# palash1992/GEM

Measured on NVIDIA H100. Metric: nodes/sec embedded at d=128, higher is better.
Workload: dtype f32

## Files before the change

gem_b200/csrc/apply_tc.cu:

```cuda
#include "tc_common.cuh"

namespace gemb {

struct ApplyTcParams {
    int64_t n;
    const float *Q;
    const float *M;
    float *Out;
    int b1, b2, ldm, ldo;
    uint32_t a_lbo;
    uint32_t a_tile;
    uint32_t b_tile;
    uint32_t raw_slot;
};

template <int TILE_M, int NPAD>
__global__ void __launch_bounds__(384, 1) apply_tc_kernel(ApplyTcParams p) {
    extern __shared__ __align__(128) char smem[];
    __shared__ __align__(8) uint64_t s_full[2], s_tile_full, s_tile_free;
    const int tid = threadIdx.x, lane = tid & 31, warp = tid >> 5;
    const int kchunks = p.b1 / 4;
    const int ksteps = p.b1 / 8;
    const uint32_t a_sbo = 128u;
    const uint32_t b_lbo = 128u;
    const uint32_t b_sbo = (uint32_t)kchunks * 128u;
    char *raw_base = smem;
    char *a_hi = smem + 2 * (size_t)p.raw_slot, *a_lo = a_hi + p.a_tile;
    char *b_hi = a_lo + p.a_tile, *b_lo = b_hi + p.b_tile;

    if (tid == 0) {
        for (int i = 0; i < 2; i++) tc::mbar_init(tc::smem_u32(&s_full[i]), 1);
        tc::mbar_init(tc::smem_u32(&s_tile_full), 4);
        tc::mbar_init(tc::smem_u32(&s_tile_free), 8);
        asm volatile("fence.mbarrier_init.release.cluster;" ::: "memory");
    }
    for (int idx = tid; idx < NPAD * kchunks; idx += blockDim.x) {
        const int nn = idx % NPAD, kc = idx / NPAD;
        float4 v = make_float4(0.f, 0.f, 0.f, 0.f);
        if (nn < p.b2) {
            const float *m = p.M + (size_t)(4 * kc) * p.ldm + nn;
            v = make_float4(__ldg(m), __ldg(m + p.ldm), __ldg(m + 2 * (size_t)p.ldm), __ldg(m + 3 * (size_t)p.ldm));
        }
        uint4 hi, lo;
        tc::split_tf32(v, hi, lo);
        const uint32_t off = (uint32_t)(nn >> 3) * b_sbo + (uint32_t)(nn & 7) * 16u + (uint32_t)kc * b_lbo;
        *(uint4 *)(b_hi + off) = hi;
        *(uint4 *)(b_lo + off) = lo;
    }
    tc::fence_proxy_async();
    __syncthreads();

    const int64_t tiles_total = (p.n + TILE_M - 1) / TILE_M;
    const int nt = (int)((tiles_total - blockIdx.x + gridDim.x - 1) / gridDim.x);
    auto tile_row0 = [&](int t) { return ((int64_t)blockIdx.x + (int64_t)t * gridDim.x) * TILE_M; };
    auto tile_rows = [&](int t) { const int64_t r0 = tile_row0(t); return (int)(p.n - r0 < TILE_M ? p.n - r0 : TILE_M); };

    if (warp >= 8) {
        auto issue = [&](int t) {
            const int slot = t & 1;
            const uint32_t bytes = (uint32_t)tile_rows(t) * (uint32_t)p.b1 * 4u;
            const uint32_t bar = tc::smem_u32(&s_full[slot]);
            tc::mbar_expect_tx(bar, bytes);
            tc::bulk_g2s(tc::smem_u32(raw_base + (size_t)slot * p.raw_slot), p.Q + tile_row0(t) * p.b1, bytes, bar);
        };
        if (tid == 256) {
            if (nt > 0) issue(0);
            if (nt > 1) issue(1);
        }
        const int ltid = tid - 256;
        for (int t = 0; t < nt; t++) {
            const int slot = t & 1;
            const char *raw = raw_base + (size_t)slot * p.raw_slot;
            tc::mbar_wait(tc::smem_u32(&s_full[slot]), (uint32_t)(t >> 1) & 1);
            if (t >= 1) tc::mbar_wait(tc::smem_u32(&s_tile_free), (uint32_t)(t - 1) & 1);
            const int vr = tile_rows(t);
            for (int idx = ltid; idx < TILE_M * kchunks; idx += 128) {
                const int m = idx / kchunks, kc = idx - m * kchunks;
                float4 v = make_float4(0.f, 0.f, 0.f, 0.f);
                if (m < vr) v = *(const float4 *)(raw + ((size_t)m * p.b1 + 4 * kc) * 4);
                uint4 hi, lo;
                tc::split_tf32(v, hi, lo);
                const uint32_t off = (uint32_t)(m >> 3) * a_sbo + (uint32_t)(m & 7) * 16u + (uint32_t)kc * p.a_lbo;
                *(uint4 *)(a_hi + off) = hi;
                *(uint4 *)(a_lo + off) = lo;
            }
            tc::fence_proxy_async();
            __syncwarp();
            if (lane == 0) tc::mbar_arrive(tc::smem_u32(&s_tile_full));
            tc::named_sync(1, 128);
            if (tid == 256 && t + 2 < nt) issue(t + 2);
        }
    } else {
        const int wg = warp >> 2;
        const bool active = wg * 64 < TILE_M;
        float acc[NPAD / 2];
        const uint32_t a_off = (uint32_t)wg * 8u * a_sbo;
        for (int t = 0; t < nt; t++) {
            tc::mbar_wait(tc::smem_u32(&s_tile_full), (uint32_t)t & 1);
            __syncwarp();
            uint64_t dah = tc::make_desc(tc::smem_u32(a_hi) + a_off, p.a_lbo, a_sbo), dal = tc::make_desc(tc::smem_u32(a_lo) + a_off, p.a_lbo, a_sbo);
            uint64_t dbh = tc::make_desc(tc::smem_u32(b_hi), b_lbo, b_sbo), dbl = tc::make_desc(tc::smem_u32(b_lo), b_lbo, b_sbo);
            const uint64_t a_step = (uint64_t)((2u * p.a_lbo) >> 4), b_step = (uint64_t)((2u * b_lbo) >> 4);
            if (active) {
                tc::wgmma_fence();
                for (int ks = 0; ks < ksteps; ks++) {
                    tc::wgmma_tf32<NPAD>(acc, dah, dbh, ks > 0 ? 1u : 0u);
                    tc::wgmma_tf32<NPAD>(acc, dah, dbl, 1u);
                    tc::wgmma_tf32<NPAD>(acc, dal, dbh, 1u);
                    dah += a_step; dal += a_step; dbh += b_step; dbl += b_step;
                }
                tc::wgmma_commit();
                tc::wgmma_wait_all();
            }
            __syncwarp();
            if (lane == 0) tc::mbar_arrive(tc::smem_u32(&s_tile_free));
            if (!active) continue;
            const int vr = tile_rows(t);
            const int r0 = wg * 64 + (warp & 3) * 16 + (lane >> 2);
            float *orow = p.Out + tile_row0(t) * p.ldo;
#pragma unroll
            for (int j = 0; j < NPAD / 8; j++) {
                const int col = j * 8 + (lane & 3) * 2;
                if (col < p.b2) {
                    if (r0 < vr) *(float2 *)(orow + (size_t)r0 * p.ldo + col) = make_float2(acc[4 * j], acc[4 * j + 1]);
                    if (r0 + 8 < vr) *(float2 *)(orow + (size_t)(r0 + 8) * p.ldo + col) = make_float2(acc[4 * j + 2], acc[4 * j + 3]);
                }
            }
        }
    }
}

template <int TILE_M, int NPAD>
static int apply_tc_launch_t(gemb_ctx *ctx, const ApplyTcParams &p, int grid, size_t smem_bytes) {
    static size_t attr_bytes = 0;
    if (attr_bytes < smem_bytes) {
        GEMB_CUDA(cudaFuncSetAttribute(apply_tc_kernel<TILE_M, NPAD>, cudaFuncAttributeMaxDynamicSharedMemorySize, (int)smem_bytes));
        attr_bytes = smem_bytes;
    }
    apply_tc_kernel<TILE_M, NPAD><<<grid, 384, smem_bytes, ctx->stream>>>(p);
    GEMB_CUDA(cudaGetLastError());
    count_launch();
    return GEMB_OK;
}

template <int TILE_M>
static int apply_tc_dispatch(gemb_ctx *ctx, const ApplyTcParams &p, int npad, int grid, size_t smem_bytes) {
    switch (npad) {
        case 32: return apply_tc_launch_t<TILE_M, 32>(ctx, p, grid, smem_bytes);
        case 64: return apply_tc_launch_t<TILE_M, 64>(ctx, p, grid, smem_bytes);
        case 80: return apply_tc_launch_t<TILE_M, 80>(ctx, p, grid, smem_bytes);
        case 96: return apply_tc_launch_t<TILE_M, 96>(ctx, p, grid, smem_bytes);
        default: return apply_tc_launch_t<TILE_M, 128>(ctx, p, grid, smem_bytes);
    }
}

static int pad_width(int b) {
    const int widths[5] = {32, 64, 80, 96, 128};
    for (int w : widths) if (w >= b) return w;
    return 128;
}

static size_t apply_smem_bytes(int tile_m, int b1, int npad) {
    const size_t raw_slot = (size_t)tile_m * b1 * 4, a_tile = (size_t)(b1 / 4) * (16 * tile_m + 16);
    const size_t b_tile = (size_t)(npad / 8) * (b1 / 4) * 128;
    return 2 * raw_slot + 2 * a_tile + 2 * b_tile + 256;
}

int apply_tc_launch(gemb_ctx *ctx, int64_t n, const float *Q, int b1, const float *M, int ldm, int b2, float *Out, int ldo) {
    if (b1 % 8 || b2 % 4 || b1 > 128 || ldo < b2 || ldo % 4 || ((uintptr_t)Out & 15) || n <= 0) return GEMB_ERR_UNSUPPORTED;
    const int cfg[5][2] = {{128, 128}, {64, 128}, {128, 64}, {64, 64}, {64, 32}};
    int tile_m = 0, nbw = 0;
    for (const auto &c : cfg) {
        const int w = std::min(c[1], b2);
        if (apply_smem_bytes(c[0], b1, pad_width(w)) <= 226 * 1024) { tile_m = c[0]; nbw = w; break; }
    }
    if (!tile_m) return GEMB_ERR_UNSUPPORTED;
    const int64_t tiles = (n + tile_m - 1) / tile_m;
    int grid = ctx->sm_count;
    if (grid > tiles) grid = (int)tiles;
    for (int n0 = 0; n0 < b2; n0 += nbw) {
        ApplyTcParams p;
        const int w = std::min(nbw, b2 - n0), npad = pad_width(w);
        p.n = n; p.Q = Q; p.M = M + n0; p.Out = Out + n0; p.b1 = b1; p.b2 = w; p.ldm = ldm; p.ldo = ldo;
        p.a_lbo = 16u * (uint32_t)tile_m + 16u;
        p.a_tile = (uint32_t)(b1 / 4) * p.a_lbo;
        p.b_tile = (uint32_t)(npad / 8) * (uint32_t)(b1 / 4) * 128u;
        p.raw_slot = (uint32_t)((size_t)tile_m * b1 * 4);
        const size_t smem_bytes = apply_smem_bytes(tile_m, b1, npad);
        if (tile_m == 128) GEMB_TRY(apply_tc_dispatch<128>(ctx, p, npad, grid, smem_bytes));
        else GEMB_TRY(apply_tc_dispatch<64>(ctx, p, npad, grid, smem_bytes));
    }
    return GEMB_OK;
}

}
```

gem_b200/csrc/gram_tc.cu:

```cuda
#include "tc_common.cuh"

namespace gemb {

struct GramTcParams {
    int64_t n;
    const float *P, *Q;
    int ldp, ldq;
    int m0, n0, mb, nb;
    double *part;
    int ldg;
    int64_t part_stride;
    int stage_rows;
    uint32_t tile_bytes_a, tile_bytes_b;
    uint32_t raw_bytes_p, raw_bytes_q;
};

__device__ __forceinline__ void transform_unit(const char *raw, int ld, int c0, int w, int valid_rows, int k4, int j32,
                                               int lane, char *tile_hi, char *tile_lo, uint32_t lbo, uint32_t sbo) {
    const int mn = j32 * 32 + lane;
    if (mn >= w) return;
    const int k0 = k4 * 4;
    const float *src = (const float *)raw + (size_t)k0 * ld + c0 + mn;
    float4 v;
    v.x = (k0 + 0 < valid_rows) ? src[0] : 0.f;
    v.y = (k0 + 1 < valid_rows) ? src[(size_t)ld] : 0.f;
    v.z = (k0 + 2 < valid_rows) ? src[2 * (size_t)ld] : 0.f;
    v.w = (k0 + 3 < valid_rows) ? src[3 * (size_t)ld] : 0.f;
    uint4 hi, lo;
    tc::split_tf32(v, hi, lo);
    const uint32_t off = (uint32_t)(mn >> 3) * sbo + (uint32_t)(mn & 7) * 16u + (uint32_t)k4 * lbo;
    *(uint4 *)(tile_hi + off) = hi;
    *(uint4 *)(tile_lo + off) = lo;
}

template <bool QRAW, bool BSEP, int NPAD>
__global__ void __launch_bounds__(384, 1) gram_tc_kernel(GramTcParams p) {
    extern __shared__ __align__(128) char smem[];
    __shared__ __align__(8) uint64_t s_full[3], s_tile_full[2], s_tile_free[2];
    const int tid = threadIdx.x, lane = tid & 31, warp = tid >> 5;
    const int kblocks = p.stage_rows / 8;
    const int kquads = p.stage_rows / 4;
    const uint32_t lbo = 128u;
    const uint32_t sbo = (uint32_t)kquads * 128u;
    const uint32_t raw_stage = p.raw_bytes_p + (QRAW ? p.raw_bytes_q : 0);
    const uint32_t stage_bytes = 2 * p.tile_bytes_a + (BSEP ? 2 * p.tile_bytes_b : 0);
    char *raw_base = smem;
    char *tile_base = smem + 3 * (size_t)raw_stage;

    if (tid == 0) {
        for (int i = 0; i < 2; i++) { tc::mbar_init(tc::smem_u32(&s_tile_full[i]), 4); tc::mbar_init(tc::smem_u32(&s_tile_free[i]), 8); }
        for (int i = 0; i < 3; i++) tc::mbar_init(tc::smem_u32(&s_full[i]), 1);
        asm volatile("fence.mbarrier_init.release.cluster;" ::: "memory");
    }
    __syncthreads();

    const int64_t stages_total = (p.n + p.stage_rows - 1) / p.stage_rows;
    const int64_t per_cta = (stages_total + gridDim.x - 1) / gridDim.x;
    const int64_t s_begin = (int64_t)blockIdx.x * per_cta;
    const int64_t s_end = s_begin + per_cta < stages_total ? s_begin + per_cta : stages_total;
    const int nst = (int)(s_end > s_begin ? s_end - s_begin : 0);

    if (warp >= 8) {
        const int lw = warp - 8;
        auto issue = [&](int it) {
            const int slot = it % 3;
            const int64_t row0 = (s_begin + it) * p.stage_rows;
            const int64_t vr = p.n - row0 < p.stage_rows ? p.n - row0 : p.stage_rows;
            const uint32_t bytes_p = (uint32_t)(vr * p.ldp * 4), bytes_q = QRAW ? (uint32_t)(vr * p.ldq * 4) : 0u;
            const uint32_t bar = tc::smem_u32(&s_full[slot]);
            char *dst = raw_base + (size_t)slot * raw_stage;
            tc::mbar_expect_tx(bar, bytes_p + bytes_q);
            tc::bulk_g2s(tc::smem_u32(dst), p.P + row0 * p.ldp, bytes_p, bar);
            if (QRAW) tc::bulk_g2s(tc::smem_u32(dst + p.raw_bytes_p), p.Q + row0 * p.ldq, bytes_q, bar);
        };
        if (tid == 256)
            for (int it = 0; it < 3 && it < nst; it++) issue(it);
        for (int it = 0; it < nst; it++) {
            const int st = it & 1, slot = it % 3;
            char *base = tile_base + (size_t)st * stage_bytes;
            const char *raw = raw_base + (size_t)slot * raw_stage;
            tc::mbar_wait(tc::smem_u32(&s_full[slot]), (uint32_t)(it / 3) & 1);
            if (it >= 2) tc::mbar_wait(tc::smem_u32(&s_tile_free[st]), (uint32_t)((it >> 1) - 1) & 1);
            const int64_t row0 = (s_begin + it) * p.stage_rows;
            const int vr = (int)(p.n - row0 < p.stage_rows ? p.n - row0 : p.stage_rows);
            const int units_a = kquads * ((p.mb + 31) / 32);
#pragma unroll 3
            for (int u = lw; u < units_a; u += 4)
                transform_unit(raw, p.ldp, p.m0, p.mb, vr, u % kquads, u / kquads, lane, base, base + p.tile_bytes_a, lbo, sbo);
            if (BSEP) {
                const int units_b = kquads * ((p.nb + 31) / 32);
                char *qb = base + 2 * p.tile_bytes_a;
                const char *rb = QRAW ? raw + p.raw_bytes_p : raw;
                const int ldb = QRAW ? p.ldq : p.ldp;
#pragma unroll 3
                for (int u = lw; u < units_b; u += 4)
                    transform_unit(rb, ldb, p.n0, p.nb, vr, u % kquads, u / kquads, lane, qb, qb + p.tile_bytes_b, lbo, sbo);
            }
            tc::fence_proxy_async();
            __syncwarp();
            if (lane == 0) tc::mbar_arrive(tc::smem_u32(&s_tile_full[st]));
            tc::named_sync(1, 128);
            if (tid == 256 && it + 3 < nst) issue(it + 3);
        }
    } else {
        const int wg = warp >> 2;
        const bool active = wg * 64 < p.mb;
        float acc[NPAD / 2], racc[NPAD / 2];
#pragma unroll
        for (int i = 0; i < NPAD / 2; i++) racc[i] = 0.f;
        for (int it = 0; it < nst; it++) {
            const int st = it & 1;
            tc::mbar_wait(tc::smem_u32(&s_tile_full[st]), (uint32_t)(it >> 1) & 1);
            if (active) {
                const uint32_t a_hi = tc::smem_u32(tile_base + (size_t)st * stage_bytes), a_lo = a_hi + p.tile_bytes_a;
                const uint32_t b_hi = BSEP ? a_hi + 2 * p.tile_bytes_a : a_hi;
                const uint32_t b_lo = BSEP ? b_hi + p.tile_bytes_b : a_lo;
                const uint32_t a_off = (uint32_t)wg * 8u * sbo;
                uint64_t dah = tc::make_desc(a_hi + a_off, lbo, sbo), dal = tc::make_desc(a_lo + a_off, lbo, sbo);
                uint64_t dbh = tc::make_desc(b_hi, lbo, sbo), dbl = tc::make_desc(b_lo, lbo, sbo);
                const uint64_t step = (uint64_t)((2u * lbo) >> 4);
                tc::wgmma_fence();
                for (int kb = 0; kb < kblocks; kb++) {
                    tc::wgmma_tf32<NPAD>(acc, dah, dbh, kb > 0 ? 1u : 0u);
                    tc::wgmma_tf32<NPAD>(acc, dah, dbl, 1u);
                    tc::wgmma_tf32<NPAD>(acc, dal, dbh, 1u);
                    dah += step; dal += step; dbh += step; dbl += step;
                }
                tc::wgmma_commit();
                tc::wgmma_wait_all();
            }
            __syncwarp();
            if (lane == 0) tc::mbar_arrive(tc::smem_u32(&s_tile_free[st]));
            if (active) {
#pragma unroll
                for (int i = 0; i < NPAD / 2; i++) racc[i] += acc[i];
            }
        }
        if (active) {
            const int r0 = wg * 64 + (warp & 3) * 16 + (lane >> 2);
            double *dst = p.part + (size_t)blockIdx.x * p.part_stride + (size_t)p.m0 * p.ldg + p.n0;
#pragma unroll
            for (int i = 0; i < NPAD / 2; i++) {
                const int row = r0 + ((i >> 1) & 1) * 8, col = (i >> 2) * 8 + (lane & 3) * 2 + (i & 1);
                if (row < p.mb && col < p.nb) dst[(size_t)row * p.ldg + col] = (double)racc[i];
            }
        }
    }
}

template <bool QRAW, bool BSEP, int NPAD>
static int gram_tc_launch_t(gemb_ctx *ctx, const GramTcParams &p, int grid, size_t smem_bytes) {
    static size_t attr_bytes = 0;
    if (attr_bytes < smem_bytes) {
        GEMB_CUDA(cudaFuncSetAttribute(gram_tc_kernel<QRAW, BSEP, NPAD>, cudaFuncAttributeMaxDynamicSharedMemorySize, (int)smem_bytes));
        attr_bytes = smem_bytes;
    }
    gram_tc_kernel<QRAW, BSEP, NPAD><<<grid, 384, smem_bytes, ctx->stream>>>(p);
    GEMB_CUDA(cudaGetLastError());
    count_launch();
    return GEMB_OK;
}

template <bool QRAW, bool BSEP>
static int gram_tc_dispatch(gemb_ctx *ctx, const GramTcParams &p, int grid, size_t smem_bytes) {
    if (p.nb <= 32) return gram_tc_launch_t<QRAW, BSEP, 32>(ctx, p, grid, smem_bytes);
    if (p.nb <= 64) return gram_tc_launch_t<QRAW, BSEP, 64>(ctx, p, grid, smem_bytes);
    if (p.nb <= 80) return gram_tc_launch_t<QRAW, BSEP, 80>(ctx, p, grid, smem_bytes);
    if (p.nb <= 96) return gram_tc_launch_t<QRAW, BSEP, 96>(ctx, p, grid, smem_bytes);
    return gram_tc_launch_t<QRAW, BSEP, 128>(ctx, p, grid, smem_bytes);
}

int gram_tc_launch(gemb_ctx *ctx, int64_t n, const float *P, int b1, const float *Q, int b2, double *G) {
    const bool cross = (P != Q);
    if (b1 % 4 || b2 % 4 || n <= 0) return GEMB_ERR_UNSUPPORTED;
    const int bm = (b1 + 127) / 128, bn = (b2 + 127) / 128;
    const size_t cols_raw = (size_t)b1 + (cross ? b2 : 0);
    size_t cols_tile = 0;
    for (int i = 0; i < bm; i++)
        for (int j = 0; j < bn; j++) {
            const int mb = std::min(128, b1 - 128 * i), nb = std::min(128, b2 - 128 * j);
            const bool bsep = cross || i != j;
            cols_tile = std::max(cols_tile, (size_t)(mb + 7) / 8 * 8 + (bsep ? (size_t)(nb + 7) / 8 * 8 : 0));
        }
    const size_t bytes_per_row = 3 * 4 * cols_raw + 2 * 2 * 4 * cols_tile;
    int rows = (int)((176 * 1024) / bytes_per_row) / 8 * 8;
    if (rows > 64) rows = 64;
    if (rows < 8) return GEMB_ERR_UNSUPPORTED;
    const size_t sbo = (size_t)(rows / 4) * 128;
    const size_t raw_stage = (size_t)rows * cols_raw * 4;
    const size_t smem_bytes = 3 * raw_stage + 2 * cols_tile / 8 * 2 * sbo + 16 * sbo + 1024;
    if (smem_bytes > 226 * 1024) return GEMB_ERR_UNSUPPORTED;
    const int64_t stages_total = (n + rows - 1) / rows;
    int grid = ctx->sm_count;
    if (grid > stages_total) grid = (int)stages_total;
    double *part = nullptr;
    GEMB_TRY(red_scratch(ctx, (size_t)grid * b1 * b2, &part));
    GramTcParams p;
    p.n = n; p.P = P; p.Q = Q; p.ldp = b1; p.ldq = b2;
    p.part = part; p.ldg = b2; p.part_stride = (int64_t)b1 * b2;
    p.stage_rows = rows;
    p.raw_bytes_p = (uint32_t)(rows * b1 * 4);
    p.raw_bytes_q = (uint32_t)(rows * b2 * 4);
    for (int i = 0; i < bm; i++)
        for (int j = 0; j < bn; j++) {
            p.m0 = 128 * i; p.mb = std::min(128, b1 - p.m0);
            p.n0 = 128 * j; p.nb = std::min(128, b2 - p.n0);
            p.tile_bytes_a = (uint32_t)((p.mb + 7) / 8) * (uint32_t)(rows / 4) * 128u;
            p.tile_bytes_b = (uint32_t)((p.nb + 7) / 8) * (uint32_t)(rows / 4) * 128u;
            if (cross) GEMB_TRY((gram_tc_dispatch<true, true>(ctx, p, grid, smem_bytes)));
            else if (i != j) GEMB_TRY((gram_tc_dispatch<false, true>(ctx, p, grid, smem_bytes)));
            else GEMB_TRY((gram_tc_dispatch<false, false>(ctx, p, grid, smem_bytes)));
        }
    return sum_partials_launch(ctx, grid, (int64_t)b1 * b2, part, G);
}

}
```

gem_b200/csrc/tc_common.cuh:

```cuda
#pragma once
#include "common.cuh"

namespace gemb {
namespace tc {

__device__ __forceinline__ uint32_t smem_u32(const void *p) { return (uint32_t)__cvta_generic_to_shared(p); }

__device__ __forceinline__ void mbar_init(uint32_t bar, uint32_t count) {
    asm volatile("mbarrier.init.shared::cta.b64 [%0], %1;" ::"r"(bar), "r"(count));
}
__device__ __forceinline__ bool mbar_try_wait(uint32_t bar, uint32_t parity) {
    uint32_t ok;
    asm volatile(
        "{\n.reg .pred p;\nmbarrier.try_wait.parity.shared::cta.b64 p, [%1], %2;\nselp.b32 %0, 1, 0, p;\n}"
        : "=r"(ok)
        : "r"(bar), "r"(parity)
        : "memory");
    return ok != 0;
}
__device__ __forceinline__ void mbar_wait(uint32_t bar, uint32_t parity) {
    for (uint32_t it = 0; it < (1u << 22); it++) {
        if (mbar_try_wait(bar, parity)) return;
        __nanosleep(40);
    }
    __trap();
}
__device__ __forceinline__ void mbar_arrive(uint32_t bar) {
    asm volatile("mbarrier.arrive.shared::cta.b64 _, [%0];" ::"r"(bar) : "memory");
}
__device__ __forceinline__ void mbar_expect_tx(uint32_t bar, uint32_t bytes) {
    asm volatile("mbarrier.arrive.expect_tx.shared::cta.b64 _, [%0], %1;" ::"r"(bar), "r"(bytes) : "memory");
}
__device__ __forceinline__ void bulk_g2s(uint32_t dst_smem, const void *src, uint32_t bytes, uint32_t bar) {
    asm volatile("cp.async.bulk.shared::cluster.global.mbarrier::complete_tx::bytes [%0], [%1], %2, [%3];"
                 ::"r"(dst_smem), "l"(src), "r"(bytes), "r"(bar) : "memory");
}
__device__ __forceinline__ void fence_proxy_async() { asm volatile("fence.proxy.async.shared::cta;" ::: "memory"); }
__device__ __forceinline__ void named_sync(uint32_t id, uint32_t count) {
    asm volatile("bar.sync %0, %1;" ::"r"(id), "r"(count) : "memory");
}

__device__ __forceinline__ uint32_t to_tf32(float x) {
    uint32_t r;
    asm("cvt.rna.tf32.f32 %0, %1;" : "=r"(r) : "f"(x));
    return r;
}
__device__ __forceinline__ void split_tf32(const float4 &v, uint4 &hi, uint4 &lo) {
    hi.x = to_tf32(v.x); hi.y = to_tf32(v.y); hi.z = to_tf32(v.z); hi.w = to_tf32(v.w);
    lo.x = to_tf32(v.x - __uint_as_float(hi.x));
    lo.y = to_tf32(v.y - __uint_as_float(hi.y));
    lo.z = to_tf32(v.z - __uint_as_float(hi.z));
    lo.w = to_tf32(v.w - __uint_as_float(hi.w));
}

__device__ __forceinline__ uint64_t make_desc(uint32_t smem_addr, uint32_t lbo_bytes, uint32_t sbo_bytes) {
    uint64_t d = 0;
    d |= (uint64_t)((smem_addr >> 4) & 0x3FFF);
    d |= (uint64_t)((lbo_bytes >> 4) & 0x3FFF) << 16;
    d |= (uint64_t)((sbo_bytes >> 4) & 0x3FFF) << 32;
    return d;
}

__device__ __forceinline__ void wgmma_fence() { asm volatile("wgmma.fence.sync.aligned;" ::: "memory"); }
__device__ __forceinline__ void wgmma_commit() { asm volatile("wgmma.commit_group.sync.aligned;" ::: "memory"); }
__device__ __forceinline__ void wgmma_wait_all() { asm volatile("wgmma.wait_group.sync.aligned 0;" ::: "memory"); }

template <int N> __device__ __forceinline__ void wgmma_tf32(float (&d)[N / 2], uint64_t a, uint64_t b, uint32_t scale_d);
template <> __device__ __forceinline__ void wgmma_tf32<32>(float (&d)[16], uint64_t a, uint64_t b, uint32_t scale_d) {
    asm volatile(
        "{\n.reg .pred p;\nsetp.ne.b32 p, %18, 0;\n"
        "wgmma.mma_async.sync.aligned.m64n32k8.f32.tf32.tf32 {"
        "%0, %1, %2, %3, %4, %5, %6, %7, %8, %9, %10, %11, %12, %13, %14, %15"
        "}, %16, %17, p, 1, 1;\n}\n"
        : "+f"(d[0]), "+f"(d[1]), "+f"(d[2]), "+f"(d[3]), "+f"(d[4]), "+f"(d[5]), "+f"(d[6]), "+f"(d[7]),
          "+f"(d[8]), "+f"(d[9]), "+f"(d[10]), "+f"(d[11]), "+f"(d[12]), "+f"(d[13]), "+f"(d[14]), "+f"(d[15])
        : "l"(a), "l"(b), "r"(scale_d));
}
template <> __device__ __forceinline__ void wgmma_tf32<64>(float (&d)[32], uint64_t a, uint64_t b, uint32_t scale_d) {
    asm volatile(
        "{\n.reg .pred p;\nsetp.ne.b32 p, %34, 0;\n"
        "wgmma.mma_async.sync.aligned.m64n64k8.f32.tf32.tf32 {"
        "%0, %1, %2, %3, %4, %5, %6, %7, %8, %9, %10, %11, %12, %13, %14, %15, "
        "%16, %17, %18, %19, %20, %21, %22, %23, %24, %25, %26, %27, %28, %29, %30, %31"
        "}, %32, %33, p, 1, 1;\n}\n"
        : "+f"(d[0]), "+f"(d[1]), "+f"(d[2]), "+f"(d[3]), "+f"(d[4]), "+f"(d[5]), "+f"(d[6]), "+f"(d[7]),
          "+f"(d[8]), "+f"(d[9]), "+f"(d[10]), "+f"(d[11]), "+f"(d[12]), "+f"(d[13]), "+f"(d[14]), "+f"(d[15]),
          "+f"(d[16]), "+f"(d[17]), "+f"(d[18]), "+f"(d[19]), "+f"(d[20]), "+f"(d[21]), "+f"(d[22]), "+f"(d[23]),
          "+f"(d[24]), "+f"(d[25]), "+f"(d[26]), "+f"(d[27]), "+f"(d[28]), "+f"(d[29]), "+f"(d[30]), "+f"(d[31])
        : "l"(a), "l"(b), "r"(scale_d));
}
template <> __device__ __forceinline__ void wgmma_tf32<80>(float (&d)[40], uint64_t a, uint64_t b, uint32_t scale_d) {
    asm volatile(
        "{\n.reg .pred p;\nsetp.ne.b32 p, %42, 0;\n"
        "wgmma.mma_async.sync.aligned.m64n80k8.f32.tf32.tf32 {"
        "%0, %1, %2, %3, %4, %5, %6, %7, %8, %9, %10, %11, %12, %13, %14, %15, "
        "%16, %17, %18, %19, %20, %21, %22, %23, %24, %25, %26, %27, %28, %29, %30, %31, "
        "%32, %33, %34, %35, %36, %37, %38, %39"
        "}, %40, %41, p, 1, 1;\n}\n"
        : "+f"(d[0]), "+f"(d[1]), "+f"(d[2]), "+f"(d[3]), "+f"(d[4]), "+f"(d[5]), "+f"(d[6]), "+f"(d[7]),
          "+f"(d[8]), "+f"(d[9]), "+f"(d[10]), "+f"(d[11]), "+f"(d[12]), "+f"(d[13]), "+f"(d[14]), "+f"(d[15]),
          "+f"(d[16]), "+f"(d[17]), "+f"(d[18]), "+f"(d[19]), "+f"(d[20]), "+f"(d[21]), "+f"(d[22]), "+f"(d[23]),
          "+f"(d[24]), "+f"(d[25]), "+f"(d[26]), "+f"(d[27]), "+f"(d[28]), "+f"(d[29]), "+f"(d[30]), "+f"(d[31]),
          "+f"(d[32]), "+f"(d[33]), "+f"(d[34]), "+f"(d[35]), "+f"(d[36]), "+f"(d[37]), "+f"(d[38]), "+f"(d[39])
        : "l"(a), "l"(b), "r"(scale_d));
}
template <> __device__ __forceinline__ void wgmma_tf32<96>(float (&d)[48], uint64_t a, uint64_t b, uint32_t scale_d) {
    asm volatile(
        "{\n.reg .pred p;\nsetp.ne.b32 p, %50, 0;\n"
        "wgmma.mma_async.sync.aligned.m64n96k8.f32.tf32.tf32 {"
        "%0, %1, %2, %3, %4, %5, %6, %7, %8, %9, %10, %11, %12, %13, %14, %15, "
        "%16, %17, %18, %19, %20, %21, %22, %23, %24, %25, %26, %27, %28, %29, %30, %31, "
        "%32, %33, %34, %35, %36, %37, %38, %39, %40, %41, %42, %43, %44, %45, %46, %47"
        "}, %48, %49, p, 1, 1;\n}\n"
        : "+f"(d[0]), "+f"(d[1]), "+f"(d[2]), "+f"(d[3]), "+f"(d[4]), "+f"(d[5]), "+f"(d[6]), "+f"(d[7]),
          "+f"(d[8]), "+f"(d[9]), "+f"(d[10]), "+f"(d[11]), "+f"(d[12]), "+f"(d[13]), "+f"(d[14]), "+f"(d[15]),
          "+f"(d[16]), "+f"(d[17]), "+f"(d[18]), "+f"(d[19]), "+f"(d[20]), "+f"(d[21]), "+f"(d[22]), "+f"(d[23]),
          "+f"(d[24]), "+f"(d[25]), "+f"(d[26]), "+f"(d[27]), "+f"(d[28]), "+f"(d[29]), "+f"(d[30]), "+f"(d[31]),
          "+f"(d[32]), "+f"(d[33]), "+f"(d[34]), "+f"(d[35]), "+f"(d[36]), "+f"(d[37]), "+f"(d[38]), "+f"(d[39]),
          "+f"(d[40]), "+f"(d[41]), "+f"(d[42]), "+f"(d[43]), "+f"(d[44]), "+f"(d[45]), "+f"(d[46]), "+f"(d[47])
        : "l"(a), "l"(b), "r"(scale_d));
}
template <> __device__ __forceinline__ void wgmma_tf32<128>(float (&d)[64], uint64_t a, uint64_t b, uint32_t scale_d) {
    asm volatile(
        "{\n.reg .pred p;\nsetp.ne.b32 p, %66, 0;\n"
        "wgmma.mma_async.sync.aligned.m64n128k8.f32.tf32.tf32 {"
        "%0, %1, %2, %3, %4, %5, %6, %7, %8, %9, %10, %11, %12, %13, %14, %15, "
        "%16, %17, %18, %19, %20, %21, %22, %23, %24, %25, %26, %27, %28, %29, %30, %31, "
        "%32, %33, %34, %35, %36, %37, %38, %39, %40, %41, %42, %43, %44, %45, %46, %47, "
        "%48, %49, %50, %51, %52, %53, %54, %55, %56, %57, %58, %59, %60, %61, %62, %63"
        "}, %64, %65, p, 1, 1;\n}\n"
        : "+f"(d[0]), "+f"(d[1]), "+f"(d[2]), "+f"(d[3]), "+f"(d[4]), "+f"(d[5]), "+f"(d[6]), "+f"(d[7]),
          "+f"(d[8]), "+f"(d[9]), "+f"(d[10]), "+f"(d[11]), "+f"(d[12]), "+f"(d[13]), "+f"(d[14]), "+f"(d[15]),
          "+f"(d[16]), "+f"(d[17]), "+f"(d[18]), "+f"(d[19]), "+f"(d[20]), "+f"(d[21]), "+f"(d[22]), "+f"(d[23]),
          "+f"(d[24]), "+f"(d[25]), "+f"(d[26]), "+f"(d[27]), "+f"(d[28]), "+f"(d[29]), "+f"(d[30]), "+f"(d[31]),
          "+f"(d[32]), "+f"(d[33]), "+f"(d[34]), "+f"(d[35]), "+f"(d[36]), "+f"(d[37]), "+f"(d[38]), "+f"(d[39]),
          "+f"(d[40]), "+f"(d[41]), "+f"(d[42]), "+f"(d[43]), "+f"(d[44]), "+f"(d[45]), "+f"(d[46]), "+f"(d[47]),
          "+f"(d[48]), "+f"(d[49]), "+f"(d[50]), "+f"(d[51]), "+f"(d[52]), "+f"(d[53]), "+f"(d[54]), "+f"(d[55]),
          "+f"(d[56]), "+f"(d[57]), "+f"(d[58]), "+f"(d[59]), "+f"(d[60]), "+f"(d[61]), "+f"(d[62]), "+f"(d[63])
        : "l"(a), "l"(b), "r"(scale_d));
}

}
}
```

Measured before the change: 14.89 million.

## Widen loader warps, deepen raw staging, add tail-8 wgmma path and n72 tile

For tiles of width 96 or less, the apply and gram kernels now use 8 loader warps instead of 4, so the TF32 hi/lo split transform gets more threads. The gram kernel sizes its raw TMA staging ring from the shared memory left over, up to 8 slots instead of a fixed 3. It also rewrites the transform loop as a flat strided item walk. When mb is 65..72, the second warpgroup computes the 8-row tail with swapped m64n8 wgmmas instead of a full 64-row tile, and a new n72 instantiation reduces padding waste. These changes add register pressure and more code paths, and the tail path has subtle index and store logic.

```diff
diff --git a/gem_b200/csrc/apply_tc.cu b/gem_b200/csrc/apply_tc.cu
--- a/gem_b200/csrc/apply_tc.cu
+++ b/gem_b200/csrc/apply_tc.cu
@@ -14,8 +14,11 @@
     uint32_t raw_slot;
 };
 
+__host__ __device__ constexpr int apply_loader_warps(int npad) { return npad <= 96 ? 8 : 4; }
+
 template <int TILE_M, int NPAD>
-__global__ void __launch_bounds__(384, 1) apply_tc_kernel(ApplyTcParams p) {
+__global__ void __launch_bounds__(256 + 32 * apply_loader_warps(NPAD), 1) apply_tc_kernel(ApplyTcParams p) {
+    constexpr int LW = apply_loader_warps(NPAD);
     extern __shared__ __align__(128) char smem[];
     __shared__ __align__(8) uint64_t s_full[2], s_tile_full, s_tile_free;
     const int tid = threadIdx.x, lane = tid & 31, warp = tid >> 5;
@@ -30,7 +33,7 @@
 
     if (tid == 0) {
         for (int i = 0; i < 2; i++) tc::mbar_init(tc::smem_u32(&s_full[i]), 1);
-        tc::mbar_init(tc::smem_u32(&s_tile_full), 4);
+        tc::mbar_init(tc::smem_u32(&s_tile_full), LW);
         tc::mbar_init(tc::smem_u32(&s_tile_free), 8);
         asm volatile("fence.mbarrier_init.release.cluster;" ::: "memory");
     }
@@ -74,7 +77,7 @@
             tc::mbar_wait(tc::smem_u32(&s_full[slot]), (uint32_t)(t >> 1) & 1);
             if (t >= 1) tc::mbar_wait(tc::smem_u32(&s_tile_free), (uint32_t)(t - 1) & 1);
             const int vr = tile_rows(t);
-            for (int idx = ltid; idx < TILE_M * kchunks; idx += 128) {
+            for (int idx = ltid; idx < TILE_M * kchunks; idx += 32 * LW) {
                 const int m = idx / kchunks, kc = idx - m * kchunks;
                 float4 v = make_float4(0.f, 0.f, 0.f, 0.f);
                 if (m < vr) v = *(const float4 *)(raw + ((size_t)m * p.b1 + 4 * kc) * 4);
@@ -87,7 +90,7 @@
             tc::fence_proxy_async();
             __syncwarp();
             if (lane == 0) tc::mbar_arrive(tc::smem_u32(&s_tile_full));
-            tc::named_sync(1, 128);
+            tc::named_sync(1, 32 * LW);
             if (tid == 256 && t + 2 < nt) issue(t + 2);
         }
     } else {
@@ -137,7 +140,7 @@
         GEMB_CUDA(cudaFuncSetAttribute(apply_tc_kernel<TILE_M, NPAD>, cudaFuncAttributeMaxDynamicSharedMemorySize, (int)smem_bytes));
         attr_bytes = smem_bytes;
     }
-    apply_tc_kernel<TILE_M, NPAD><<<grid, 384, smem_bytes, ctx->stream>>>(p);
+    apply_tc_kernel<TILE_M, NPAD><<<grid, 256 + 32 * apply_loader_warps(NPAD), smem_bytes, ctx->stream>>>(p);
     GEMB_CUDA(cudaGetLastError());
     count_launch();
     return GEMB_OK;
diff --git a/gem_b200/csrc/gram_tc.cu b/gem_b200/csrc/gram_tc.cu
--- a/gem_b200/csrc/gram_tc.cu
+++ b/gem_b200/csrc/gram_tc.cu
@@ -11,32 +11,42 @@
     int ldg;
     int64_t part_stride;
     int stage_rows;
+    int nraw;
     uint32_t tile_bytes_a, tile_bytes_b;
     uint32_t raw_bytes_p, raw_bytes_q;
 };
 
-__device__ __forceinline__ void transform_unit(const char *raw, int ld, int c0, int w, int valid_rows, int k4, int j32,
-                                               int lane, char *tile_hi, char *tile_lo, uint32_t lbo, uint32_t sbo) {
-    const int mn = j32 * 32 + lane;
-    if (mn >= w) return;
-    const int k0 = k4 * 4;
-    const float *src = (const float *)raw + (size_t)k0 * ld + c0 + mn;
-    float4 v;
-    v.x = (k0 + 0 < valid_rows) ? src[0] : 0.f;
-    v.y = (k0 + 1 < valid_rows) ? src[(size_t)ld] : 0.f;
-    v.z = (k0 + 2 < valid_rows) ? src[2 * (size_t)ld] : 0.f;
-    v.w = (k0 + 3 < valid_rows) ? src[3 * (size_t)ld] : 0.f;
-    uint4 hi, lo;
-    tc::split_tf32(v, hi, lo);
-    const uint32_t off = (uint32_t)(mn >> 3) * sbo + (uint32_t)(mn & 7) * 16u + (uint32_t)k4 * lbo;
-    *(uint4 *)(tile_hi + off) = hi;
-    *(uint4 *)(tile_lo + off) = lo;
-}
-
-template <bool QRAW, bool BSEP, int NPAD>
-__global__ void __launch_bounds__(384, 1) gram_tc_kernel(GramTcParams p) {
+__device__ __forceinline__ void transform_items(const char *raw, int ld, int c0, int w, int kquads, int valid_rows, int t,
+                                                int nt, char *tile_hi, char *tile_lo, uint32_t lbo, uint32_t sbo) {
+    const int dm = nt % w, dk = nt / w;
+    int mn = t % w, k4 = t / w;
+#pragma unroll 2
+    for (; k4 < kquads;) {
+        const int k0 = k4 * 4;
+        const float *src = (const float *)raw + (size_t)k0 * ld + c0 + mn;
+        float4 v;
+        v.x = (k0 + 0 < valid_rows) ? src[0] : 0.f;
+        v.y = (k0 + 1 < valid_rows) ? src[(size_t)ld] : 0.f;
+        v.z = (k0 + 2 < valid_rows) ? src[2 * (size_t)ld] : 0.f;
+        v.w = (k0 + 3 < valid_rows) ? src[3 * (size_t)ld] : 0.f;
+        uint4 hi, lo;
+        tc::split_tf32(v, hi, lo);
+        const uint32_t off = (uint32_t)(mn >> 3) * sbo + (uint32_t)(mn & 7) * 16u + (uint32_t)k4 * lbo;
+        *(uint4 *)(tile_hi + off) = hi;
+        *(uint4 *)(tile_lo + off) = lo;
+        mn += dm; k4 += dk;
+        if (mn >= w) { mn -= w; k4++; }
+    }
+}
+
+constexpr int GRAM_MAX_RAW = 8;
+__host__ __device__ constexpr int gram_loader_warps(int npad) { return npad <= 96 ? 8 : 4; }
+
+template <bool QRAW, bool BSEP, int NPAD, bool TAIL8>
+__global__ void __launch_bounds__(256 + 32 * gram_loader_warps(NPAD), 1) gram_tc_kernel(GramTcParams p) {
+    constexpr int LW = gram_loader_warps(NPAD);
     extern __shared__ __align__(128) char smem[];
-    __shared__ __align__(8) uint64_t s_full[3], s_tile_full[2], s_tile_free[2];
+    __shared__ __align__(8) uint64_t s_full[GRAM_MAX_RAW], s_tile_full[2], s_tile_free[2];
     const int tid = threadIdx.x, lane = tid & 31, warp = tid >> 5;
     const int kblocks = p.stage_rows / 8;
     const int kquads = p.stage_rows / 4;
@@ -45,11 +55,12 @@
     const uint32_t raw_stage = p.raw_bytes_p + (QRAW ? p.raw_bytes_q : 0);
     const uint32_t stage_bytes = 2 * p.tile_bytes_a + (BSEP ? 2 * p.tile_bytes_b : 0);
     char *raw_base = smem;
-    char *tile_base = smem + 3 * (size_t)raw_stage;
+    const int nraw = p.nraw;
+    char *tile_base = smem + (size_t)nraw * raw_stage;
 
     if (tid == 0) {
-        for (int i = 0; i < 2; i++) { tc::mbar_init(tc::smem_u32(&s_tile_full[i]), 4); tc::mbar_init(tc::smem_u32(&s_tile_free[i]), 8); }
-        for (int i = 0; i < 3; i++) tc::mbar_init(tc::smem_u32(&s_full[i]), 1);
+        for (int i = 0; i < 2; i++) { tc::mbar_init(tc::smem_u32(&s_tile_full[i]), LW); tc::mbar_init(tc::smem_u32(&s_tile_free[i]), 8); }
+        for (int i = 0; i < nraw; i++) tc::mbar_init(tc::smem_u32(&s_full[i]), 1);
         asm volatile("fence.mbarrier_init.release.cluster;" ::: "memory");
     }
     __syncthreads();
@@ -61,9 +72,8 @@
     const int nst = (int)(s_end > s_begin ? s_end - s_begin : 0);
 
     if (warp >= 8) {
-        const int lw = warp - 8;
         auto issue = [&](int it) {
-            const int slot = it % 3;
+            const int slot = it % nraw;
             const int64_t row0 = (s_begin + it) * p.stage_rows;
             const int64_t vr = p.n - row0 < p.stage_rows ? p.n - row0 : p.stage_rows;
             const uint32_t bytes_p = (uint32_t)(vr * p.ldp * 4), bytes_q = QRAW ? (uint32_t)(vr * p.ldq * 4) : 0u;
@@ -74,37 +84,73 @@
             if (QRAW) tc::bulk_g2s(tc::smem_u32(dst + p.raw_bytes_p), p.Q + row0 * p.ldq, bytes_q, bar);
         };
         if (tid == 256)
-            for (int it = 0; it < 3 && it < nst; it++) issue(it);
+            for (int it = 0; it < nraw && it < nst; it++) issue(it);
         for (int it = 0; it < nst; it++) {
-            const int st = it & 1, slot = it % 3;
+            const int st = it & 1, slot = it % nraw;
             char *base = tile_base + (size_t)st * stage_bytes;
             const char *raw = raw_base + (size_t)slot * raw_stage;
-            tc::mbar_wait(tc::smem_u32(&s_full[slot]), (uint32_t)(it / 3) & 1);
+            tc::mbar_wait(tc::smem_u32(&s_full[slot]), (uint32_t)(it / nraw) & 1);
             if (it >= 2) tc::mbar_wait(tc::smem_u32(&s_tile_free[st]), (uint32_t)((it >> 1) - 1) & 1);
             const int64_t row0 = (s_begin + it) * p.stage_rows;
             const int vr = (int)(p.n - row0 < p.stage_rows ? p.n - row0 : p.stage_rows);
-            const int units_a = kquads * ((p.mb + 31) / 32);
-#pragma unroll 3
-            for (int u = lw; u < units_a; u += 4)
-                transform_unit(raw, p.ldp, p.m0, p.mb, vr, u % kquads, u / kquads, lane, base, base + p.tile_bytes_a, lbo, sbo);
+            transform_items(raw, p.ldp, p.m0, p.mb, kquads, vr, tid - 256, 32 * LW, base, base + p.tile_bytes_a, lbo, sbo);
             if (BSEP) {
-                const int units_b = kquads * ((p.nb + 31) / 32);
                 char *qb = base + 2 * p.tile_bytes_a;
-                const char *rb = QRAW ? raw + p.raw_bytes_p : raw;
-                const int ldb = QRAW ? p.ldq : p.ldp;
-#pragma unroll 3
-                for (int u = lw; u < units_b; u += 4)
-                    transform_unit(rb, ldb, p.n0, p.nb, vr, u % kquads, u / kquads, lane, qb, qb + p.tile_bytes_b, lbo, sbo);
+                transform_items(QRAW ? raw + p.raw_bytes_p : raw, QRAW ? p.ldq : p.ldp, p.n0, p.nb, kquads, vr, tid - 256,
+                                32 * LW, qb, qb + p.tile_bytes_b, lbo, sbo);
             }
             tc::fence_proxy_async();
             __syncwarp();
             if (lane == 0) tc::mbar_arrive(tc::smem_u32(&s_tile_full[st]));
-            tc::named_sync(1, 128);
-            if (tid == 256 && it + 3 < nst) issue(it + 3);
+            tc::named_sync(1, 32 * LW);
+            if (tid == 256 && it + nraw < nst) issue(it + nraw);
         }
     } else {
         const int wg = warp >> 2;
         const bool active = wg * 64 < p.mb;
+        if (TAIL8 && wg == 1) {
+            const bool two = p.nb > 64;
+            const int c1 = two ? (p.nb + 7) / 8 * 8 - 64 : 0;
+            float t0[4], t1[4], r0[4] = {0.f, 0.f, 0.f, 0.f}, r1[4] = {0.f, 0.f, 0.f, 0.f};
+            for (int it = 0; it < nst; it++) {
+                const int st = it & 1;
+                tc::mbar_wait(tc::smem_u32(&s_tile_full[st]), (uint32_t)(it >> 1) & 1);
+                const uint32_t a_hi = tc::smem_u32(tile_base + (size_t)st * stage_bytes), a_lo = a_hi + p.tile_bytes_a;
+                const uint32_t b_hi = BSEP ? a_hi + 2 * p.tile_bytes_a : a_hi;
+                const uint32_t b_lo = BSEP ? b_hi + p.tile_bytes_b : a_lo;
+                const uint32_t r_off = 8u * sbo, c_off = (uint32_t)(c1 / 8) * sbo;
+                uint64_t drh = tc::make_desc(a_hi + r_off, lbo, sbo), drl = tc::make_desc(a_lo + r_off, lbo, sbo);
+                uint64_t d0h = tc::make_desc(b_hi, lbo, sbo), d0l = tc::make_desc(b_lo, lbo, sbo);
+                uint64_t d1h = tc::make_desc(b_hi + c_off, lbo, sbo), d1l = tc::make_desc(b_lo + c_off, lbo, sbo);
+                const uint64_t step = (uint64_t)((2u * lbo) >> 4);
+                tc::wgmma_fence();
+                for (int kb = 0; kb < kblocks; kb++) {
+                    tc::wgmma_tf32<8>(t0, d0h, drh, kb > 0 ? 1u : 0u);
+                    tc::wgmma_tf32<8>(t0, d0l, drh, 1u);
+                    tc::wgmma_tf32<8>(t0, d0h, drl, 1u);
+                    if (two) {
+                        tc::wgmma_tf32<8>(t1, d1h, drh, kb > 0 ? 1u : 0u);
+                        tc::wgmma_tf32<8>(t1, d1l, drh, 1u);
+                        tc::wgmma_tf32<8>(t1, d1h, drl, 1u);
+                    }
+                    drh += step; drl += step; d0h += step; d0l += step; d1h += step; d1l += step;
+                }
+                tc::wgmma_commit();
+                tc::wgmma_wait_all();
+                __syncwarp();
+                if (lane == 0) tc::mbar_arrive(tc::smem_u32(&s_tile_free[st]));
+#pragma unroll
+                for (int i = 0; i < 4; i++) { r0[i] += t0[i]; if (two) r1[i] += t1[i]; }
+            }
+            double *dst = p.part + (size_t)blockIdx.x * p.part_stride + (size_t)p.m0 * p.ldg + p.n0;
+#pragma unroll
+            for (int i = 0; i < 4; i++) {
+                const int row = 64 + (lane & 3) * 2 + (i & 1), cm = (warp & 3) * 16 + (lane >> 2) + (i >> 1) * 8;
+                if (row < p.mb && cm < p.nb) dst[(size_t)row * p.ldg + cm] = (double)r0[i];
+                if (two && row < p.mb && c1 + cm >= 64 && c1 + cm < p.nb) dst[(size_t)row * p.ldg + c1 + cm] = (double)r1[i];
+            }
+            return;
+        }
         float acc[NPAD / 2], racc[NPAD / 2];
 #pragma unroll
         for (int i = 0; i < NPAD / 2; i++) racc[i] = 0.f;
@@ -148,26 +194,33 @@
     }
 }
 
-template <bool QRAW, bool BSEP, int NPAD>
+template <bool QRAW, bool BSEP, int NPAD, bool TAIL8>
 static int gram_tc_launch_t(gemb_ctx *ctx, const GramTcParams &p, int grid, size_t smem_bytes) {
     static size_t attr_bytes = 0;
     if (attr_bytes < smem_bytes) {
-        GEMB_CUDA(cudaFuncSetAttribute(gram_tc_kernel<QRAW, BSEP, NPAD>, cudaFuncAttributeMaxDynamicSharedMemorySize, (int)smem_bytes));
+        GEMB_CUDA(cudaFuncSetAttribute(gram_tc_kernel<QRAW, BSEP, NPAD, TAIL8>, cudaFuncAttributeMaxDynamicSharedMemorySize, (int)smem_bytes));
         attr_bytes = smem_bytes;
     }
-    gram_tc_kernel<QRAW, BSEP, NPAD><<<grid, 384, smem_bytes, ctx->stream>>>(p);
+    gram_tc_kernel<QRAW, BSEP, NPAD, TAIL8><<<grid, 256 + 32 * gram_loader_warps(NPAD), smem_bytes, ctx->stream>>>(p);
     GEMB_CUDA(cudaGetLastError());
     count_launch();
     return GEMB_OK;
 }
 
+template <bool QRAW, bool BSEP, bool TAIL8>
+static int gram_tc_dispatch_n(gemb_ctx *ctx, const GramTcParams &p, int grid, size_t smem_bytes) {
+    if (p.nb <= 32) return gram_tc_launch_t<QRAW, BSEP, 32, TAIL8>(ctx, p, grid, smem_bytes);
+    if (p.nb <= 64) return gram_tc_launch_t<QRAW, BSEP, 64, TAIL8>(ctx, p, grid, smem_bytes);
+    if (p.nb <= 72) return gram_tc_launch_t<QRAW, BSEP, 72, TAIL8>(ctx, p, grid, smem_bytes);
+    if (p.nb <= 80) return gram_tc_launch_t<QRAW, BSEP, 80, TAIL8>(ctx, p, grid, smem_bytes);
+    if (p.nb <= 96) return gram_tc_launch_t<QRAW, BSEP, 96, TAIL8>(ctx, p, grid, smem_bytes);
+    return gram_tc_launch_t<QRAW, BSEP, 128, TAIL8>(ctx, p, grid, smem_bytes);
+}
+
 template <bool QRAW, bool BSEP>
 static int gram_tc_dispatch(gemb_ctx *ctx, const GramTcParams &p, int grid, size_t smem_bytes) {
-    if (p.nb <= 32) return gram_tc_launch_t<QRAW, BSEP, 32>(ctx, p, grid, smem_bytes);
-    if (p.nb <= 64) return gram_tc_launch_t<QRAW, BSEP, 64>(ctx, p, grid, smem_bytes);
-    if (p.nb <= 80) return gram_tc_launch_t<QRAW, BSEP, 80>(ctx, p, grid, smem_bytes);
-    if (p.nb <= 96) return gram_tc_launch_t<QRAW, BSEP, 96>(ctx, p, grid, smem_bytes);
-    return gram_tc_launch_t<QRAW, BSEP, 128>(ctx, p, grid, smem_bytes);
+    if (p.mb > 64 && p.mb <= 72) return gram_tc_dispatch_n<QRAW, BSEP, true>(ctx, p, grid, smem_bytes);
+    return gram_tc_dispatch_n<QRAW, BSEP, false>(ctx, p, grid, smem_bytes);
 }
 
 int gram_tc_launch(gemb_ctx *ctx, int64_t n, const float *P, int b1, const float *Q, int b2, double *G) {
@@ -188,8 +241,10 @@
     if (rows < 8) return GEMB_ERR_UNSUPPORTED;
     const size_t sbo = (size_t)(rows / 4) * 128;
     const size_t raw_stage = (size_t)rows * cols_raw * 4;
-    const size_t smem_bytes = 3 * raw_stage + 2 * cols_tile / 8 * 2 * sbo + 16 * sbo + 1024;
-    if (smem_bytes > 226 * 1024) return GEMB_ERR_UNSUPPORTED;
+    const size_t fixed_bytes = 2 * cols_tile / 8 * 2 * sbo + 16 * sbo + 1024;
+    if (3 * raw_stage + fixed_bytes > 226 * 1024) return GEMB_ERR_UNSUPPORTED;
+    const int nraw = (int)std::min<size_t>(GRAM_MAX_RAW, (226 * 1024 - fixed_bytes) / raw_stage);
+    const size_t smem_bytes = (size_t)nraw * raw_stage + fixed_bytes;
     const int64_t stages_total = (n + rows - 1) / rows;
     int grid = ctx->sm_count;
     if (grid > stages_total) grid = (int)stages_total;
@@ -199,6 +254,7 @@
     p.n = n; p.P = P; p.Q = Q; p.ldp = b1; p.ldq = b2;
     p.part = part; p.ldg = b2; p.part_stride = (int64_t)b1 * b2;
     p.stage_rows = rows;
+    p.nraw = nraw;
     p.raw_bytes_p = (uint32_t)(rows * b1 * 4);
     p.raw_bytes_q = (uint32_t)(rows * b2 * 4);
     for (int i = 0; i < bm; i++)
diff --git a/gem_b200/csrc/tc_common.cuh b/gem_b200/csrc/tc_common.cuh
--- a/gem_b200/csrc/tc_common.cuh
+++ b/gem_b200/csrc/tc_common.cuh
@@ -66,6 +66,13 @@
 __device__ __forceinline__ void wgmma_wait_all() { asm volatile("wgmma.wait_group.sync.aligned 0;" ::: "memory"); }
 
 template <int N> __device__ __forceinline__ void wgmma_tf32(float (&d)[N / 2], uint64_t a, uint64_t b, uint32_t scale_d);
+template <> __device__ __forceinline__ void wgmma_tf32<8>(float (&d)[4], uint64_t a, uint64_t b, uint32_t scale_d) {
+    asm volatile(
+        "{\n.reg .pred p;\nsetp.ne.b32 p, %6, 0;\n"
+        "wgmma.mma_async.sync.aligned.m64n8k8.f32.tf32.tf32 {%0, %1, %2, %3}, %4, %5, p, 1, 1;\n}\n"
+        : "+f"(d[0]), "+f"(d[1]), "+f"(d[2]), "+f"(d[3])
+        : "l"(a), "l"(b), "r"(scale_d));
+}
 template <> __device__ __forceinline__ void wgmma_tf32<32>(float (&d)[16], uint64_t a, uint64_t b, uint32_t scale_d) {
     asm volatile(
         "{\n.reg .pred p;\nsetp.ne.b32 p, %18, 0;\n"
@@ -87,6 +94,21 @@
           "+f"(d[8]), "+f"(d[9]), "+f"(d[10]), "+f"(d[11]), "+f"(d[12]), "+f"(d[13]), "+f"(d[14]), "+f"(d[15]),
           "+f"(d[16]), "+f"(d[17]), "+f"(d[18]), "+f"(d[19]), "+f"(d[20]), "+f"(d[21]), "+f"(d[22]), "+f"(d[23]),
           "+f"(d[24]), "+f"(d[25]), "+f"(d[26]), "+f"(d[27]), "+f"(d[28]), "+f"(d[29]), "+f"(d[30]), "+f"(d[31])
+        : "l"(a), "l"(b), "r"(scale_d));
+}
+template <> __device__ __forceinline__ void wgmma_tf32<72>(float (&d)[36], uint64_t a, uint64_t b, uint32_t scale_d) {
+    asm volatile(
+        "{\n.reg .pred p;\nsetp.ne.b32 p, %38, 0;\n"
+        "wgmma.mma_async.sync.aligned.m64n72k8.f32.tf32.tf32 {"
+        "%0, %1, %2, %3, %4, %5, %6, %7, %8, %9, %10, %11, %12, %13, %14, %15, "
+        "%16, %17, %18, %19, %20, %21, %22, %23, %24, %25, %26, %27, %28, %29, %30, %31, "
+        "%32, %33, %34, %35"
+        "}, %36, %37, p, 1, 1;\n}\n"
+        : "+f"(d[0]), "+f"(d[1]), "+f"(d[2]), "+f"(d[3]), "+f"(d[4]), "+f"(d[5]), "+f"(d[6]), "+f"(d[7]),
+          "+f"(d[8]), "+f"(d[9]), "+f"(d[10]), "+f"(d[11]), "+f"(d[12]), "+f"(d[13]), "+f"(d[14]), "+f"(d[15]),
+          "+f"(d[16]), "+f"(d[17]), "+f"(d[18]), "+f"(d[19]), "+f"(d[20]), "+f"(d[21]), "+f"(d[22]), "+f"(d[23]),
+          "+f"(d[24]), "+f"(d[25]), "+f"(d[26]), "+f"(d[27]), "+f"(d[28]), "+f"(d[29]), "+f"(d[30]), "+f"(d[31]),
+          "+f"(d[32]), "+f"(d[33]), "+f"(d[34]), "+f"(d[35])
         : "l"(a), "l"(b), "r"(scale_d));
 }
 template <> __device__ __forceinline__ void wgmma_tf32<80>(float (&d)[40], uint64_t a, uint64_t b, uint32_t scale_d) {
```

Result: faster. 15.60 million (median of 6 runs) (+4.7%).
